# nrclaudio/spVIPES

Measured on AMD Instinct MI355X. Metric: cells/sec/training-step (2-group PoE VAE), higher is better.
Workload: dtype bf16

## Files before the change

include/spvipes_hip.h:

```cpp
#ifndef SPVIPES_HIP_H
#define SPVIPES_HIP_H

#include <stdint.h>

#ifdef __cplusplus
extern "C" {
#endif

#define SPV_OK 0
#define SPV_ERR_ARG (-1)
#define SPV_ERR_LAUNCH (-2)
#define SPV_ERR_UNSUPPORTED (-3)

#define SPV_COUNT_F32 0
#define SPV_COUNT_U16 1

#define SPV_NB_CMAX 64
#define SPV_DEC_KP 16
#define SPV_DEC_KS 32
#define SPV_DEC_KP_WIDE 32
#define SPV_DEC_KS_WIDE 64
#define SPV_DEC_CELLS_PER_WG 128

int spv_version(void);
// ... 263 lines not shown
int spv_bn_bwd(const spv_bn_batch* a, void* stream);

typedef struct spv_sample_prob {
  const float* post; int32_t n;
  const float* eps;
  float* scale; float* logz; float* theta; float* kl;
  const float* g_loc; const float* g_logvar; const float* g_scale; const float* g_logz; const float* g_kl;
  float* d_post;
  int64_t g_ld;
} spv_sample_prob;
typedef struct spv_sample_batch { spv_sample_prob p[SPV_MAXP]; int32_t nprob, B; } spv_sample_batch;
int spv_enc_sample_fwd(const spv_sample_batch* a, void* stream);
int spv_enc_sample_bwd(const spv_sample_batch* a, void* stream);
int spv_enc_heads_fwd(const spv_bn_batch* bn, const spv_sample_batch* sb, void* stream);
int spv_enc_heads_bwd(const spv_bn_batch* bn, const spv_sample_batch* sb, void* stream);

#define SPV_NB_GSPL_MAX 160
#define SPV_POE_LMAX 1024

int spv_poe_partner(const float* labels0, const float* labels1, int32_t B0, int32_t B1, int32_t* order0, int32_t* order1,
                    int32_t* rank0, int32_t* rank1, int32_t* tables, int32_t* partner0, int32_t* mode0,
                    int32_t* partner1, int32_t* mode1, int32_t* err, void* stream);

int spv_poe_rank(const float* labels0, const float* labels1, int32_t B0, int32_t B1, int32_t* order0, int32_t* order1,
                 int32_t* rank0, int32_t* rank1, int32_t* tables, int32_t* err, void* stream);

typedef struct spv_poe_args {
  const float* stats[2]; int64_t ld[2];
  const int32_t* partner[2]; const int32_t* mode[2];
  const float* eps[2];
// ... 121 lines not shown
```

spvipes_amd/_abi.py:

```python
from __future__ import annotations

import ctypes as C
import os
from typing import NamedTuple, Optional

import torch

_HERE = os.path.dirname(os.path.abspath(__file__))
LIB_PATH = os.path.join(_HERE, "_lib", "libspvipes_hip.so")

SPV_COUNT_F32, SPV_COUNT_U16 = 0, 1
NB_CMAX, DEC_KP, DEC_KS, DEC_CELLS_PER_WG = 64, 16, 32, 128
DEC_KPS = DEC_KP + DEC_KS


class DecSlots(NamedTuple):
    kslots: int
    KP: int
    KS: int
    KPS: int


DEC_NARROW = DecSlots(0, DEC_KP, DEC_KS, DEC_KPS)
DEC_WIDE = DecSlots(1, 32, 64, 96)
# ... 58 lines not shown


class SpvBnBatch(C.Structure):
    _fields_ = [("p", SpvBnProb * SPV_MAXP), ("nprob", C.c_int32), ("B", C.c_int32), ("training", C.c_int32), ("relu", C.c_int32),
                ("eps", C.c_float), ("momentum", C.c_float)]


class SpvSampleProb(C.Structure):
    _fields_ = [("post", C.c_void_p), ("n", C.c_int32), ("eps", C.c_void_p), ("scale", C.c_void_p), ("logz", C.c_void_p), ("theta", C.c_void_p),
                ("kl", C.c_void_p), ("g_loc", C.c_void_p), ("g_logvar", C.c_void_p), ("g_scale", C.c_void_p), ("g_logz", C.c_void_p),
                ("g_kl", C.c_void_p), ("d_post", C.c_void_p), ("g_ld", C.c_int64)]


class SpvSampleBatch(C.Structure):
    _fields_ = [("p", SpvSampleProb * SPV_MAXP), ("nprob", C.c_int32), ("B", C.c_int32)]


class SpvPoeArgs(C.Structure):
    _fields_ = [("stats", C.c_void_p * 2), ("ld", C.c_int64 * 2), ("partner", C.c_void_p * 2), ("mode", C.c_void_p * 2), ("eps", C.c_void_p * 2),
                ("loc", C.c_void_p * 2), ("logvar", C.c_void_p * 2), ("scale", C.c_void_p * 2), ("logz", C.c_void_p * 2), ("theta", C.c_void_p * 2),
                ("kl", C.c_void_p * 2), ("g_loc", C.c_void_p * 2), ("g_logvar", C.c_void_p * 2), ("g_scale", C.c_void_p * 2),
                ("g_logz", C.c_void_p * 2), ("g_kl", C.c_void_p * 2), ("d_stats", C.c_void_p * 2), ("B", C.c_int32 * 2), ("n", C.c_int32),
                ("clamp_scale", C.c_int32), ("lone_passthrough", C.c_int32), ("expert", C.c_void_p * 2), ("ld_expert", C.c_int64 * 2),
                ("d_expert", C.c_void_p * 2), ("lab", C.c_void_p * 2), ("order", C.c_void_p * 2), ("rank", C.c_void_p * 2), ("tables", C.c_void_p)]


SPV_POE_MAXG, POE_COMP_SEG, POE_COMP_CMAX = 4, 16, 64


class SpvFc1FwdArgs(C.Structure):
# ... 174 lines not shown
    "spv_dec_tables_grouped": (C.c_int, [C.POINTER(SpvDecGroup), C.c_int32, C.c_void_p]),
    "spv_dec_logits_grouped": (C.c_int, [C.POINTER(SpvDecGroup), C.c_int32, C.c_void_p]),
    "spv_dec_lse_grouped": (C.c_int, [C.POINTER(SpvDecGroup), C.c_int32, C.c_void_p]),
    "spv_dec_nb_fwd_grouped": (C.c_int, [C.POINTER(SpvDecGroup), C.c_int32, C.c_int32, C.c_void_p]),
    "spv_dec_heads_bwd_grouped": (C.c_int, [C.POINTER(SpvDecGroup), C.c_int32, C.c_void_p]),
    "spv_gemm_bf16_grouped": (C.c_int, [C.POINTER(SpvGemmArgs), C.c_int32, C.c_void_p]),
    "spv_linear_fwd": (C.c_int, [C.POINTER(SpvLinearBatch), C.c_void_p]),
    "spv_linear_dgrad": (C.c_int, [C.POINTER(SpvLinearBatch), C.c_void_p]),
    "spv_linear_wgrad": (C.c_int, [C.POINTER(SpvLinearBatch), C.c_void_p, C.c_int64, C.c_void_p]),
    "spv_bn_fwd": (C.c_int, [C.POINTER(SpvBnBatch), C.c_void_p]),
    "spv_bn_bwd": (C.c_int, [C.POINTER(SpvBnBatch), C.c_void_p]),
    "spv_enc_sample_fwd": (C.c_int, [C.POINTER(SpvSampleBatch), C.c_void_p]),
    "spv_enc_sample_bwd": (C.c_int, [C.POINTER(SpvSampleBatch), C.c_void_p]),
    "spv_enc_heads_fwd": (C.c_int, [C.POINTER(SpvBnBatch), C.POINTER(SpvSampleBatch), C.c_void_p]),
    "spv_enc_heads_bwd": (C.c_int, [C.POINTER(SpvBnBatch), C.POINTER(SpvSampleBatch), C.c_void_p]),
    "spv_poe_partner": (C.c_int, [C.c_void_p, C.c_void_p, C.c_int32, C.c_int32, C.c_void_p, C.c_void_p, C.c_void_p, C.c_void_p, C.c_void_p,
                                  C.c_void_p, C.c_void_p, C.c_void_p, C.c_void_p, C.c_void_p, C.c_void_p]),
    "spv_poe_rank": (C.c_int, [C.c_void_p, C.c_void_p, C.c_int32, C.c_int32, C.c_void_p, C.c_void_p, C.c_void_p, C.c_void_p, C.c_void_p, C.c_void_p, C.c_void_p]),
    "spv_poe_fuse_fwd": (C.c_int, [C.POINTER(SpvPoeArgs), C.c_void_p]),
    "spv_poe_fuse_bwd": (C.c_int, [C.POINTER(SpvPoeArgs), C.c_void_p]),
    "spv_plan_invmap": (C.c_int, [C.c_void_p, C.c_int32, C.c_void_p, C.c_int32, C.c_void_p, C.c_int32, C.c_void_p, C.c_int32, C.c_void_p]),
    "spv_plan_argmax": (C.c_int, [C.POINTER(SpvPlan), C.c_void_p, C.c_void_p, C.c_void_p, C.c_void_p, C.c_int32, C.c_int32, C.c_void_p,
                                  C.c_void_p, C.c_void_p]),
    "spv_plan_expert_fwd": (C.c_int, [C.POINTER(SpvPlanExpertArgs), C.c_void_p]),
    "spv_plan_expert_bwd": (C.c_int, [C.POINTER(SpvPlanExpertArgs), C.c_void_p]),
    "spv_poe_comp_fwd": (C.c_int, [C.POINTER(SpvPoeCompArgs), C.c_void_p]),
    "spv_poe_comp_bwd": (C.c_int, [C.POINTER(SpvPoeCompArgs), C.c_void_p]),
    "spv_zsplit_fwd": (C.c_int, [C.POINTER(SpvZsplitArgs), C.c_void_p]),
    "spv_zsplit_bwd": (C.c_int, [C.POINTER(SpvZsplitArgs), C.c_void_p]),
    "spv_bn_fold_fwd": (C.c_int, [C.POINTER(SpvFoldBatch), C.c_void_p]),
# ... 96 lines not shown
```

spvipes_amd/build.py:

```python
from __future__ import annotations

import os
import shutil
import subprocess
import sys

HERE = os.path.dirname(os.path.abspath(__file__))
CSRC = os.path.join(HERE, "csrc")
LIBDIR = os.path.join(HERE, "_lib")
LIB = os.path.join(LIBDIR, "libspvipes_hip.so")
SOURCES = ["spv_abi.hip"]
HEADERS = ["spv_common.h", "spv_gemm.h", "spv_fc1.h", "spv_dec_gemm.h", "spv_decoder.h", "spv_dec_expected.h", "spv_de.h", "spv_de_median.h", "spv_small.h", "spv_poe_n.h", os.path.join("..", "..", "include", "spvipes_hip.h")]


FLAGS = [
    "--offload-arch=gfx950", "-O3", "-std=c++17", "-fPIC", "-shared", "-Wno-unused-value",
    "-fno-slp-vectorize",
]


def build_id() -> str:
    import hashlib

    h = hashlib.sha256()
    h.update(" ".join(FLAGS).encode())
    for name in sorted(SOURCES + HEADERS):
        with open(os.path.join(CSRC, name), "rb") as f:
# ... 44 lines not shown
```

spvipes_amd/csrc/spv_abi.hip:

```cpp
#include "../../include/spvipes_hip.h"
#include "spv_common.h"
#include "spv_gemm.h"
#include "spv_fc1.h"
#include "spv_dec_gemm.h"
#include "spv_decoder.h"
#include "spv_dec_expected.h"
#include "spv_de.h"
#include "spv_de_median.h"
#include "spv_small.h"
#include "spv_poe_n.h"

#include <cstdio>
#include <cstdlib>
#include <cstring>

using namespace spv;

static thread_local char g_err[512] = "";
static int fail(int code, const char* fmt, const char* what = "") {
  snprintf(g_err, sizeof(g_err), fmt, what);
  return code;
}
static int launch_status(const char* what) {
  hipError_t e = hipGetLastError();
// ... 1215 lines not shown
    if (q0.Y != sb->p[e].post || q1.Y != sb->p[e].post + n || q0.ldy != 2 * n || q1.ldy != 2 * n)
      return fail(SPV_ERR_ARG, "%s: the BatchNorm outputs must be the two halves of the sampling problem's post [B][2n]", who);
  }
  return SPV_OK;
}
extern "C" int spv_enc_heads_fwd(const spv_bn_batch* bn, const spv_sample_batch* sb, void* stream) {
  int rc = check_heads(bn, sb, "spv_enc_heads_fwd");
  if (rc) return rc;
  for (int i = 0; i < sb->nprob; ++i) if (!sb->p[i].logz || !sb->p[i].theta || !sb->p[i].kl) return fail(SPV_ERR_ARG, "spv_enc_heads_fwd: null output%s");
  hipStream_t s = (hipStream_t)stream;
  const unsigned nb = (bn->B + BN_ROWS - 1) / BN_ROWS;
  if (bn->training) hipLaunchKernelGGL(bn_stats_kernel, dim3(nb, bn->nprob), dim3(256), 0, s, *bn);
  hipLaunchKernelGGL(enc_heads_bn_sample_fwd_kernel, dim3(nb, sb->nprob), dim3(256), 0, s, *bn, *sb);
  return launch_status("spv_enc_heads_fwd");
}
extern "C" int spv_enc_heads_bwd(const spv_bn_batch* bn, const spv_sample_batch* sb, void* stream) {
  int rc = check_heads(bn, sb, "spv_enc_heads_bwd");
  if (rc) return rc;
  for (int i = 0; i < sb->nprob; ++i) if (!sb->p[i].d_post) return fail(SPV_ERR_ARG, "spv_enc_heads_bwd: null output%s");
  for (int i = 0; i < bn->nprob; ++i) {
    const spv_bn_prob& q = bn->p[i];
    if (!q.dX || !q.dgamma || !q.dbeta) return fail(SPV_ERR_ARG, "spv_enc_heads_bwd: null pointer%s");
    const int e = i / 2, n = sb->p[e].n;
    if (q.dY != sb->p[e].d_post + (i & 1) * n || q.lddy != 2 * n) return fail(SPV_ERR_ARG, "spv_enc_heads_bwd: dY must be the halves of d_post [B][2n]%s");
  }
  if (!bn->training) return fail(SPV_ERR_UNSUPPORTED, "spv_enc_heads_bwd: training-mode BatchNorm only (use spv_enc_sample_bwd + spv_bn_bwd)%s");
  hipStream_t s = (hipStream_t)stream;
  const unsigned nb = (bn->B + BN_ROWS - 1) / BN_ROWS;
  hipLaunchKernelGGL(enc_heads_bwd_reduce_kernel, dim3(nb, sb->nprob), dim3(256), 0, s, *bn, *sb);
  hipLaunchKernelGGL(bn_bwd_apply_fin_kernel, dim3(nb, bn->nprob), dim3(256), 0, s, *bn);
// ... 805 lines not shown
```

spvipes_amd/nn_ops.py:

```python
from __future__ import annotations

import ctypes as C
from typing import List, Optional, Sequence

import torch

from . import _abi
from ._abi import SpvBnBatch, SpvLinearBatch, SpvSampleBatch, ptr, stream_ptr


def _lin_batch(B: int, relu: bool = False, drop_p: float = 0.0, seed=0, accumulate: bool = False) -> SpvLinearBatch:
    b = SpvLinearBatch()
    b.nprob, b.B, b.relu, b.drop_p, b.accumulate = 0, B, int(relu), float(drop_p), int(accumulate)
    if isinstance(seed, torch.Tensor):
        b.seed, b.seed_ptr = 0, seed.data_ptr()
    else:
        b.seed, b.seed_ptr = int(seed), None
    return b


def _add_lin(b: SpvLinearBatch, *, N: int, K: int, W=None, X=None, ldx=0, bias=None, Y=None, ldy=0, dY=None, lddy=0, dX=None, lddx=0,
             dW=None, db=None, keep=None, W2=None, n_w2=0) -> None:
    q = b.p[b.nprob]
    q.X, q.ldx, q.W, q.bias, q.Y, q.ldy, q.keep, q.W2, q.n_w2 = X, ldx, W, bias, Y, ldy, keep, W2, n_w2
# ... 25 lines not shown


class EncoderSpec:

    def __init__(self, enc, h1_group: int, h1_col: int):
        self.enc, self.h1_group, self.h1_col = enc, h1_group, h1_col
        self.n = enc.n_topics

    def params(self) -> List[torch.Tensor]:
        e = self.enc
        return [e.fc2.weight, e.fc2.bias, e.mu_encoder[0].weight, e.mu_encoder[0].bias, e.lvar_encoder[0].weight, e.lvar_encoder[0].bias,
                e.mu_encoder[1].weight, e.mu_encoder[1].bias, e.lvar_encoder[1].weight, e.lvar_encoder[1].bias]


N_ENC_PARAMS = 10


class EncoderTails(torch.autograd.Function):

    @staticmethod
    def forward(ctx, specs: Sequence[EncoderSpec], eps: Sequence[torch.Tensor], training: bool, drop_p: float, seed: int, ws, masks, *tensors):
        ctx.set_materialize_grads(False)
        n_groups = max(s.h1_group for s in specs) + 1
        h1 = tensors[:n_groups]
        par = [tensors[n_groups + i * N_ENC_PARAMS: n_groups + (i + 1) * N_ENC_PARAMS] for i in range(len(specs))]
        B, H = h1[0].shape[0], specs[0].enc.fc2.weight.shape[0]
        dev = h1[0].device
        for t in h1:
            if t.dtype != torch.float32 or not t.is_contiguous():
                raise _abi.SpvError("EncoderTails expects contiguous fp32 h1")
        new = lambda *s: torch.empty(*s, dtype=torch.float32, device=dev)
        h2 = [new(B, H) for _ in specs]
        pre = [new(B, 2 * s.n) for s in specs]
        post = [new(B, 2 * s.n) for s in specs]
        stats = [new(2, s.n, 2) for s in specs]
        nblk = -(-B // _abi.BN_ROWS)
        dp = float(drop_p) if training else 0.0
        b = _lin_batch(B, relu=True, drop_p=dp, seed=seed)
        keep_masks = []
        for i, (s, p, y) in enumerate(zip(specs, par, h2)):
            mk = None
            if masks is not None and masks[i] is not None and dp > 0:
                mk = masks[i].to(dev, torch.float32).contiguous()
                if mk.shape != (B, H):
                    raise _abi.SpvError("dropout mask must be [B, n_hidden]")
                keep_masks.append(mk)
            _add_lin(b, N=H, K=H, W=ptr(p[0]), bias=ptr(p[1]), X=_fptr(h1[s.h1_group], s.h1_col), ldx=h1[s.h1_group].shape[1], Y=ptr(y), ldy=H, keep=ptr(mk))
        _abi.call("spv_linear_fwd", C.byref(b), stream_ptr())
        b = _lin_batch(B)
        for s, p, x, y in zip(specs, par, h2, pre):
            _add_lin(b, N=s.n, K=H, W=ptr(p[2]), bias=ptr(p[3]), X=ptr(x), ldx=H, Y=_fptr(y, 0), ldy=2 * s.n)
            _add_lin(b, N=s.n, K=H, W=ptr(p[4]), bias=ptr(p[5]), X=ptr(x), ldx=H, Y=_fptr(y, s.n), ldy=2 * s.n)
        _abi.call("spv_linear_fwd", C.byref(b), stream_ptr())
        bn = SpvBnBatch()
        bn.nprob, bn.B, bn.training, bn.relu, bn.eps, bn.momentum = 0, B, int(training), 0, 1e-5, 0.1
        parts = []
        for s, p, x, y, st in zip(specs, par, pre, post, stats):
            for half, (g, be, mod) in enumerate(((p[6], p[7], s.enc.mu_encoder[1]), (p[8], p[9], s.enc.lvar_encoder[1]))):
                part = ws.get(f"tail_bn_part_{len(parts)}", (nblk, s.n, 2), torch.float32)
                parts.append(part)
                q = bn.p[bn.nprob]
                q.X, q.ldx, q.Y, q.ldy = _fptr(x, half * s.n), 2 * s.n, _fptr(y, half * s.n), 2 * s.n
                q.gamma, q.beta, q.running_mean, q.running_var = ptr(g), ptr(be), ptr(mod.running_mean), ptr(mod.running_var)
                q.stats, q.part, q.N = ptr(st[half]), ptr(part), s.n
                bn.nprob += 1
        scale = [new(B, s.n) for s in specs]
        logz = [new(B, s.n) for s in specs]
        theta = [new(B, s.n) for s in specs]
        kl = [new(B) for _ in specs]
        sb = SpvSampleBatch()
        sb.nprob, sb.B = len(specs), B
        for i, s in enumerate(specs):
            q = sb.p[i]
            q.post, q.n, q.eps, q.scale, q.logz, q.theta, q.kl = ptr(post[i]), s.n, ptr(eps[i].contiguous()), ptr(scale[i]), ptr(logz[i]), ptr(theta[i]), ptr(kl[i])
        _abi.call("spv_enc_heads_fwd", C.byref(bn), C.byref(sb), stream_ptr())
        ctx.specs, ctx.training, ctx.dp, ctx.seed, ctx.ws, ctx.n_groups, ctx.B, ctx.H = specs, training, dp, seed, ws, n_groups, B, H
        ctx.eps = [e.contiguous() for e in eps]
        ctx.save_for_backward(*tensors, *h2, *pre, *post, *stats, *scale)
        outs = []
        for i, s in enumerate(specs):
            outs += [post[i][:, :s.n], post[i][:, s.n:], scale[i], logz[i], theta[i], kl[i]]
            ctx.mark_non_differentiable(theta[i])
        return tuple(outs)

    @staticmethod
    def backward(ctx, *g):
        specs, B, H, ws, n_groups = ctx.specs, ctx.B, ctx.H, ctx.ws, ctx.n_groups
        E = len(specs)
        saved = ctx.saved_tensors
        n_in = n_groups + E * N_ENC_PARAMS
# ... 33 lines not shown
        k = 0
        for i, (s, p) in enumerate(zip(specs, par)):
            for half, (gam, be, mod) in enumerate(((p[6], p[7], s.enc.mu_encoder[1]), (p[8], p[9], s.enc.lvar_encoder[1]))):
                q = bn.p[bn.nprob]
                q.X, q.ldx, q.Y, q.ldy = _fptr(pre[i], half * s.n), 2 * s.n, _fptr(post[i], half * s.n), 2 * s.n
                q.gamma, q.beta, q.running_mean, q.running_var = ptr(gam), ptr(be), ptr(mod.running_mean), ptr(mod.running_var)
                q.stats, q.part, q.N = ptr(stats[i][half]), ptr(ws.get(f"tail_bn_part_{k}", (nblk, s.n, 2), torch.float32)), s.n
                q.dY, q.lddy, q.dX, q.lddx = _fptr(d_post[i], half * s.n), 2 * s.n, _fptr(d_pre[i], half * s.n), 2 * s.n
                q.dgamma, q.dbeta = ptr(d_gb[i][2 * half]), ptr(d_gb[i][2 * half + 1])
                bn.nprob += 1
                k += 1
        if fused:
            _abi.call("spv_enc_heads_bwd", C.byref(bn), C.byref(sb), stream_ptr())
        else:
            _abi.call("spv_bn_bwd", C.byref(bn), stream_ptr())
        dWmu, dbmu, dWlv, dblv = ([pg[i][2][0] for i in range(E)], [pg[i][3][0] for i in range(E)], [pg[i][4][0] for i in range(E)], [pg[i][5][0] for i in range(E)])
        b = _lin_batch(B)
        for i, s in enumerate(specs):
            _add_lin(b, N=s.n, K=H, W=ptr(par[i][2]), X=ptr(h2[i]), ldx=H, dY=_fptr(d_pre[i], 0), lddy=2 * s.n, dW=ptr(dWmu[i]), db=ptr(dbmu[i]))
            _add_lin(b, N=s.n, K=H, W=ptr(par[i][4]), X=ptr(h2[i]), ldx=H, dY=_fptr(d_pre[i], s.n), lddy=2 * s.n, dW=ptr(dWlv[i]), db=ptr(dblv[i]))
        from . import ops as _ops
        wsw = ws if not isinstance(ws, (list, tuple)) else ws[0]
        _wgrad(b, wsw)
        dh2 = [new(B, H) for _ in specs]
        b = _lin_batch(B)
        for i, s in enumerate(specs):
            _add_lin(b, N=2 * s.n, K=H, W=ptr(par[i][2]), W2=ptr(par[i][4]), n_w2=s.n, dY=ptr(d_pre[i]), lddy=2 * s.n, dX=ptr(dh2[i]), lddx=H)
        _abi.call("spv_linear_dgrad", C.byref(b), stream_ptr())
        dW2, db2 = [pg[i][0][0] for i in range(E)], [pg[i][1][0] for i in range(E)]
        covered = [sorted((s.h1_col, s.h1_col + H) for s in specs if s.h1_group == k) for k in range(n_groups)]
        full = [bool(c) and c[0][0] == 0 and c[-1][1] == h1[k].shape[1] and all(c[i][1] == c[i + 1][0] for i in range(len(c) - 1))
                for k, c in enumerate(covered)]
        dh1 = [torch.empty_like(t) if full[k] else torch.zeros_like(t) for k, t in enumerate(h1)]
        bw = _lin_batch(B, relu=True, drop_p=ctx.dp)
        bd = _lin_batch(B, relu=True, drop_p=ctx.dp)
        for i, s in enumerate(specs):
            x, ldx = _fptr(h1[s.h1_group], s.h1_col), h1[s.h1_group].shape[1]
            _add_lin(bw, N=H, K=H, W=ptr(par[i][0]), X=x, ldx=ldx, Y=ptr(h2[i]), ldy=H, dY=ptr(dh2[i]), lddy=H, dW=ptr(dW2[i]), db=ptr(db2[i]))
            _add_lin(bd, N=H, K=H, W=ptr(par[i][0]), Y=ptr(h2[i]), ldy=H, dY=ptr(dh2[i]), lddy=H, dX=_fptr(dh1[s.h1_group], s.h1_col), lddx=ldx)
        _wgrad(bw, wsw)
        _abi.call("spv_linear_dgrad", C.byref(bd), stream_ptr())
        grads: List[Optional[torch.Tensor]] = list(dh1)
        for i in range(E):
            grads += [pg[i][j][1] for j in range(N_ENC_PARAMS)]
        return (None, None, None, None, None, None, None, *grads)


def _loc_logvar_block(loc: torch.Tensor, logvar: torch.Tensor):
    n = loc.shape[1]
    if (loc.dtype == torch.float32 and loc.stride(1) == 1 and logvar.stride(1) == 1 and loc.stride(0) == logvar.stride(0)
            and logvar.data_ptr() == loc.data_ptr() + 4 * n and loc.stride(0) >= 2 * n):
        return loc, loc.data_ptr(), loc.stride(0)
    blk = torch.cat([loc, logvar], dim=1).contiguous()
    return blk, blk.data_ptr(), 2 * n


# ... 295 lines not shown
```

spvipes_amd/ops.py:

```python
from __future__ import annotations

import ctypes as C
import os
from dataclasses import dataclass
from typing import Dict, Optional, Tuple

import torch

from . import _abi
from ._abi import DEC_CELLS_PER_WG, NB_CMAX, SpvCounts, SpvDecParams, check, ptr, round_up, stream_ptr

N_HIDDEN_MIX = 256


@dataclass
class GroupCounts:

    X: torch.Tensor
    G: int
    col_off: int = 0
    resident: bool = False

    def __post_init__(self):
        self._xb = None
# ... 253 lines not shown
DEC_PAIR_SPLITS = os.environ.get("SPV_DEC_PAIR_SPLITS", "1") != "0"
HEADS_DMA = os.environ.get("SPV_HEADS_DMA", "1") != "0"
FUSED_HEADS = os.environ.get("SPV_FUSED_HEADS", "1") != "0"
GSPLIT_WANT = int(os.environ.get("SPV_GSPLIT_WANT", "512"))
FUSED_HEADS_F32 = os.environ.get("SPV_FUSED_HEADS_F32", "1") != "0"
FUSED_DZ = os.environ.get("SPV_FUSED_DZ", "1") != "0"
FUSED_DZ_F32 = os.environ.get("SPV_FUSED_DZ_F32", "1") != "0"
DA_FIXUP = os.environ.get("SPV_DA_FIXUP", "0")
TRUNK_FOLD = os.environ.get("SPV_TRUNK_FOLD", "1") != "0"
FUSED_PACK = os.environ.get("SPV_FUSED_PACK", "1") != "0"
DEFER_WM = os.environ.get("SPV_DEFER_WM", "1") != "0"
DEFER_BC = os.environ.get("SPV_DEFER_BC", "1") != "0"
DZ_ONLY = os.environ.get("SPV_DZ_ONLY", "0") != "0"
FWD_GROUP_STREAMS = os.environ.get("SPV_FWD_GROUP_STREAMS", "1") != "0"
BWD_GROUP_STREAMS = os.environ.get("SPV_BWD_GROUP_STREAMS", "1") != "0"
_PENDING: list = []
_PENDING_KEEP: list = []


def defer(stream, keep=()) -> None:
    if stream not in _PENDING:
        _PENDING.append(stream)
    _PENDING_KEEP.extend(keep)


def join_all_side_streams(device) -> None:
    dev = torch.device(device)
    cur = torch.cuda.current_stream(dev)
    capturing = torch.cuda.is_current_stream_capturing()
    for (idx, _i), st in _SIDE_STREAMS.items():
# ... 277 lines not shown
```

Before: 6.221 million.

## Fuse encoder tail fc2 and mu/logvar heads into one kernel with BN partials

Adds a fused encoder-tail forward kernel that computes the hidden linear (ReLU and dropout), both mean and log-variance heads, and per-block batch-norm partial statistics in one launch, keeping h2 in shared memory. A matching backward kernel chains the head dgrad and the hidden-layer dgrad through LDS. The goal is to cut launches and global round-trips of intermediates in the small-H encoder tail. It is limited to H in 64/128/256 and head width up to 32, falling back to the old path otherwise, and it uses FP32 MFMA.

```diff
diff --git a/include/spvipes_hip.h b/include/spvipes_hip.h
--- a/include/spvipes_hip.h
+++ b/include/spvipes_hip.h
@@ -301,6 +301,29 @@
 int spv_enc_sample_bwd(const spv_sample_batch* a, void* stream);
 int spv_enc_heads_fwd(const spv_bn_batch* bn, const spv_sample_batch* sb, void* stream);
 int spv_enc_heads_bwd(const spv_bn_batch* bn, const spv_sample_batch* sb, void* stream);
+int spv_enc_heads_fwd_from_partials(const spv_bn_batch* bn, const spv_sample_batch* sb, void* stream);
+
+#define SPV_TAIL_MAXE 4
+typedef struct spv_enc_tail_prob {
+  const float* h1; int64_t ldh1;
+  const float* W2; const float* b2;
+  const float* Wmu; const float* bmu; const float* Wlv; const float* blv;
+  float* h2;
+  float* pre;
+  float* part_mu; float* part_lv;
+  const float* d_pre;
+  float* dh2;
+  float* dh1; int64_t lddh1;
+  int32_t n;
+} spv_enc_tail_prob;
+typedef struct spv_enc_tail_batch {
+  spv_enc_tail_prob p[SPV_TAIL_MAXE];
+  int32_t nprob, B, H;
+  float drop_p;
+  uint64_t seed; const uint64_t* seed_ptr;
+} spv_enc_tail_batch;
+int spv_enc_tail_fwd(const spv_enc_tail_batch* a, void* stream);
+int spv_enc_tail_bwd(const spv_enc_tail_batch* a, void* stream);
 
 #define SPV_NB_GSPL_MAX 160
 #define SPV_POE_LMAX 1024
diff --git a/spvipes_amd/_abi.py b/spvipes_amd/_abi.py
--- a/spvipes_amd/_abi.py
+++ b/spvipes_amd/_abi.py
@@ -96,6 +96,20 @@
 
 class SpvSampleBatch(C.Structure):
     _fields_ = [("p", SpvSampleProb * SPV_MAXP), ("nprob", C.c_int32), ("B", C.c_int32)]
+
+
+SPV_TAIL_MAXE = 4
+
+
+class SpvEncTailProb(C.Structure):
+    _fields_ = [("h1", C.c_void_p), ("ldh1", C.c_int64), ("W2", C.c_void_p), ("b2", C.c_void_p), ("Wmu", C.c_void_p), ("bmu", C.c_void_p),
+                ("Wlv", C.c_void_p), ("blv", C.c_void_p), ("h2", C.c_void_p), ("pre", C.c_void_p), ("part_mu", C.c_void_p), ("part_lv", C.c_void_p),
+                ("d_pre", C.c_void_p), ("dh2", C.c_void_p), ("dh1", C.c_void_p), ("lddh1", C.c_int64), ("n", C.c_int32)]
+
+
+class SpvEncTailBatch(C.Structure):
+    _fields_ = [("p", SpvEncTailProb * SPV_TAIL_MAXE), ("nprob", C.c_int32), ("B", C.c_int32), ("H", C.c_int32), ("drop_p", C.c_float),
+                ("seed", C.c_uint64), ("seed_ptr", C.c_void_p)]
 
 
 class SpvPoeArgs(C.Structure):
@@ -300,6 +314,9 @@
     "spv_enc_sample_bwd": (C.c_int, [C.POINTER(SpvSampleBatch), C.c_void_p]),
     "spv_enc_heads_fwd": (C.c_int, [C.POINTER(SpvBnBatch), C.POINTER(SpvSampleBatch), C.c_void_p]),
     "spv_enc_heads_bwd": (C.c_int, [C.POINTER(SpvBnBatch), C.POINTER(SpvSampleBatch), C.c_void_p]),
+    "spv_enc_heads_fwd_from_partials": (C.c_int, [C.POINTER(SpvBnBatch), C.POINTER(SpvSampleBatch), C.c_void_p]),
+    "spv_enc_tail_fwd": (C.c_int, [C.POINTER(SpvEncTailBatch), C.c_void_p]),
+    "spv_enc_tail_bwd": (C.c_int, [C.POINTER(SpvEncTailBatch), C.c_void_p]),
     "spv_poe_partner": (C.c_int, [C.c_void_p, C.c_void_p, C.c_int32, C.c_int32, C.c_void_p, C.c_void_p, C.c_void_p, C.c_void_p, C.c_void_p,
                                   C.c_void_p, C.c_void_p, C.c_void_p, C.c_void_p, C.c_void_p, C.c_void_p]),
     "spv_poe_rank": (C.c_int, [C.c_void_p, C.c_void_p, C.c_int32, C.c_int32, C.c_void_p, C.c_void_p, C.c_void_p, C.c_void_p, C.c_void_p, C.c_void_p, C.c_void_p]),
diff --git a/spvipes_amd/build.py b/spvipes_amd/build.py
--- a/spvipes_amd/build.py
+++ b/spvipes_amd/build.py
@@ -10,7 +10,7 @@
 LIBDIR = os.path.join(HERE, "_lib")
 LIB = os.path.join(LIBDIR, "libspvipes_hip.so")
 SOURCES = ["spv_abi.hip"]
-HEADERS = ["spv_common.h", "spv_gemm.h", "spv_fc1.h", "spv_dec_gemm.h", "spv_decoder.h", "spv_dec_expected.h", "spv_de.h", "spv_de_median.h", "spv_small.h", "spv_poe_n.h", os.path.join("..", "..", "include", "spvipes_hip.h")]
+HEADERS = ["spv_common.h", "spv_gemm.h", "spv_fc1.h", "spv_dec_gemm.h", "spv_decoder.h", "spv_dec_expected.h", "spv_de.h", "spv_de_median.h", "spv_small.h", "spv_enc_tail.h", "spv_poe_n.h", os.path.join("..", "..", "include", "spvipes_hip.h")]
 
 
 FLAGS = [
diff --git a/spvipes_amd/csrc/spv_abi.hip b/spvipes_amd/csrc/spv_abi.hip
--- a/spvipes_amd/csrc/spv_abi.hip
+++ b/spvipes_amd/csrc/spv_abi.hip
@@ -8,6 +8,7 @@
 #include "spv_de.h"
 #include "spv_de_median.h"
 #include "spv_small.h"
+#include "spv_enc_tail.h"
 #include "spv_poe_n.h"
 
 #include <cstdio>
@@ -1253,6 +1254,53 @@
   hipLaunchKernelGGL(enc_heads_bn_sample_fwd_kernel, dim3(nb, sb->nprob), dim3(256), 0, s, *bn, *sb);
   return launch_status("spv_enc_heads_fwd");
 }
+extern "C" int spv_enc_heads_fwd_from_partials(const spv_bn_batch* bn, const spv_sample_batch* sb, void* stream) {
+  int rc = check_heads(bn, sb, "spv_enc_heads_fwd_from_partials");
+  if (rc) return rc;
+  for (int i = 0; i < sb->nprob; ++i) if (!sb->p[i].logz || !sb->p[i].theta || !sb->p[i].kl) return fail(SPV_ERR_ARG, "spv_enc_heads_fwd_from_partials: null output%s");
+  if (!bn->training) return fail(SPV_ERR_ARG, "spv_enc_heads_fwd_from_partials: training-mode statistics only%s");
+  const unsigned nb = (bn->B + BN_ROWS - 1) / BN_ROWS;
+  hipLaunchKernelGGL(enc_heads_bn_sample_fwd_kernel, dim3(nb, sb->nprob), dim3(256), 0, (hipStream_t)stream, *bn, *sb);
+  return launch_status("spv_enc_heads_fwd_from_partials");
+}
+
+static int check_tail(const spv_enc_tail_batch* a, const char* who, bool bwd) {
+  if (!a || a->nprob <= 0 || a->nprob > SPV_TAIL_MAXE || a->B <= 0) return fail(SPV_ERR_ARG, "%s: bad batch", who);
+  if (a->drop_p < 0.f || a->drop_p >= 1.f) return fail(SPV_ERR_ARG, "%s: dropout probability outside [0,1)", who);
+  if (a->H != 64 && a->H != 128 && a->H != 256) return fail(SPV_ERR_UNSUPPORTED, "%s: H must be 64, 128 or 256", who);
+  for (int i = 0; i < a->nprob; ++i) {
+    const spv_enc_tail_prob& q = a->p[i];
+    if (q.n <= 0 || q.n > 32) return fail(SPV_ERR_UNSUPPORTED, "%s: head width outside 1..32", who);
+    if (!q.W2 || !q.Wmu || !q.Wlv || !q.h2) return fail(SPV_ERR_ARG, "%s: null pointer", who);
+    if (bwd ? (!q.d_pre || !q.dh2 || !q.dh1 || q.lddh1 < a->H)
+            : (!q.h1 || !q.b2 || !q.bmu || !q.blv || !q.pre || q.ldh1 < a->H || (q.part_mu == nullptr) != (q.part_lv == nullptr)))
+      return fail(SPV_ERR_ARG, "%s: bad problem", who);
+    const uintptr_t al = (uintptr_t)q.W2 | (uintptr_t)q.Wmu | (uintptr_t)q.Wlv | (bwd ? 0 : ((uintptr_t)q.h1 | (uintptr_t)(q.ldh1 * 4)));
+    if (al & 15) return fail(SPV_ERR_UNSUPPORTED, "%s: operands must be 16-byte aligned", who);
+  }
+  return SPV_OK;
+}
+extern "C" int spv_enc_tail_fwd(const spv_enc_tail_batch* a, void* stream) {
+  int rc = check_tail(a, "spv_enc_tail_fwd", false);
+  if (rc) return rc;
+  hipStream_t s = (hipStream_t)stream;
+  const unsigned E = a->nprob;
+  if (a->H == 64) hipLaunchKernelGGL(enc_tail_fwd_kernel<64>, dim3((a->B + ENC_TAIL_ROWS<64> - 1) / ENC_TAIL_ROWS<64>, E), dim3(256), 0, s, *a);
+  else if (a->H == 128) hipLaunchKernelGGL(enc_tail_fwd_kernel<128>, dim3((a->B + ENC_TAIL_ROWS<128> - 1) / ENC_TAIL_ROWS<128>, E), dim3(256), 0, s, *a);
+  else hipLaunchKernelGGL(enc_tail_fwd_kernel<256>, dim3((a->B + ENC_TAIL_ROWS<256> - 1) / ENC_TAIL_ROWS<256>, E), dim3(256), 0, s, *a);
+  return launch_status("spv_enc_tail_fwd");
+}
+extern "C" int spv_enc_tail_bwd(const spv_enc_tail_batch* a, void* stream) {
+  int rc = check_tail(a, "spv_enc_tail_bwd", true);
+  if (rc) return rc;
+  hipStream_t s = (hipStream_t)stream;
+  const unsigned E = a->nprob;
+  if (a->H == 64) hipLaunchKernelGGL(enc_tail_bwd_kernel<64>, dim3((a->B + ENC_TAIL_ROWS<64> - 1) / ENC_TAIL_ROWS<64>, E), dim3(256), 0, s, *a);
+  else if (a->H == 128) hipLaunchKernelGGL(enc_tail_bwd_kernel<128>, dim3((a->B + ENC_TAIL_ROWS<128> - 1) / ENC_TAIL_ROWS<128>, E), dim3(256), 0, s, *a);
+  else hipLaunchKernelGGL(enc_tail_bwd_kernel<256>, dim3((a->B + ENC_TAIL_ROWS<256> - 1) / ENC_TAIL_ROWS<256>, E), dim3(256), 0, s, *a);
+  return launch_status("spv_enc_tail_bwd");
+}
+
 extern "C" int spv_enc_heads_bwd(const spv_bn_batch* bn, const spv_sample_batch* sb, void* stream) {
   int rc = check_heads(bn, sb, "spv_enc_heads_bwd");
   if (rc) return rc;
diff --git a/spvipes_amd/csrc/spv_enc_tail.h b/spvipes_amd/csrc/spv_enc_tail.h
--- /dev/null
+++ b/spvipes_amd/csrc/spv_enc_tail.h
@@ -0,0 +1,237 @@
+#pragma once
+#include "spv_small.h"
+
+namespace spv {
+
+typedef spv_enc_tail_prob EncTailProb;
+typedef spv_enc_tail_batch EncTailBatch;
+
+template <int H> constexpr int ENC_TAIL_ROWS = (H <= 64) ? 64 : 32;
+
+__device__ __forceinline__ void issue_fence() { __builtin_amdgcn_sched_barrier(0); }
+
+__device__ const uint64_t g_spv_zero64 = 0;
+
+__device__ __forceinline__ void ld8v(const float* p, float (&v)[8]) {
+  const f4v a = *reinterpret_cast<const f4v*>(p), b = *reinterpret_cast<const f4v*>(p + 4);
+#pragma unroll
+  for (int j = 0; j < 4; ++j) { v[j] = a[j]; v[4 + j] = b[j]; }
+}
+
+template <int H>
+__global__ __launch_bounds__(256) void enc_tail_fwd_kernel(EncTailBatch a) {
+  constexpr int TR = ENC_TAIL_ROWS<H>, RH = TR / 32, CW = 4 / RH, NT = (H / 32) / CW, KS = H / 16, LDH = H + 4, LDP = 65, NCMB = 2 * RH;
+  static_assert(BN_ROWS == 32 && (H / 32) % CW == 0, "tile shape");
+  __shared__ __attribute__((aligned(16))) float s_h2[TR * LDH];
+  __shared__ float s_pre[TR * LDP], s_acc[NCMB][256], s_mean[NCMB][32];
+  const EncTailProb& q = a.p[blockIdx.y];
+  const int lane = threadIdx.x & 63, wave = threadIdx.x >> 6, h = lane >> 5, r = lane & 31;
+  const int rh = wave / CW, cw = wave % CW;
+  const int t0 = blockIdx.x * TR;
+  const int n = q.n;
+  const float* xr = q.h1 + (long)min(t0 + 32 * rh + r, a.B - 1) * q.ldh1 + 8 * h;
+  float xa[KS][8];
+#pragma unroll
+  for (int s = 0; s < KS; ++s) ld8v(xr + 16 * s, xa[s]);
+  issue_fence();
+  const int hr = wave >> 1, half = wave & 1;
+  const float* whr = (half ? q.Wlv : q.Wmu) + (long)min(r, n - 1) * H + 8 * h;
+  const float hbias = (half ? q.blv : q.bmu)[min(r, n - 1)];
+  float wh[KS][8];
+  const uint64_t seed_add = *(a.seed_ptr ? a.seed_ptr : &g_spv_zero64);
+#pragma unroll
+  for (int t = 0; t < NT; ++t) {
+    const int col = 32 * (cw + CW * t) + r;
+    const float* wr = q.W2 + (long)col * H + 8 * h;
+    float wb[KS][8];
+#pragma unroll
+    for (int s = 0; s < KS; ++s) ld8v(wr + 16 * s, wb[s]);
+    const float bias = q.b2[col];
+    if (t == NT - 1 && hr < RH) {
+#pragma unroll
+      for (int s = 0; s < KS; ++s) ld8v(whr + 16 * s, wh[s]);
+    }
+    issue_fence();
+    f16v acc;
+#pragma unroll
+    for (int i = 0; i < 16; ++i) acc[i] = 0.f;
+#pragma unroll
+    for (int s = 0; s < KS; ++s) {
+#pragma unroll
+      for (int j = 0; j < 8; ++j) acc = mfma_f32(xa[s][j], wb[s][j], acc);
+    }
+#pragma unroll
+    for (int i = 0; i < 16; ++i) {
+      const int rl = 32 * rh + crow(i, h), b = t0 + rl;
+      float v = acc[i] + bias;
+      v = fmaxf(v, 0.f);
+      if (a.drop_p > 0.f) {
+        const bool keep = dropout_keep(a.seed + seed_add, blockIdx.y, (long)b * H + col, a.drop_p);
+        v = keep ? v * (1.0f / (1.0f - a.drop_p)) : 0.f;
+      }
+      s_h2[rl * LDH + col] = v;
+      if (b < a.B) q.h2[(long)b * H + col] = v;
+    }
+  }
+  lds_barrier();
+  if (hr < RH) {
+    const float* xs = s_h2 + (32 * hr + r) * LDH + 8 * h;
+    f16v acc;
+#pragma unroll
+    for (int i = 0; i < 16; ++i) acc[i] = 0.f;
+#pragma unroll
+    for (int s = 0; s < KS; ++s) {
+      float x[8];
+      ld8v(xs + 16 * s, x);
+#pragma unroll
+      for (int j = 0; j < 8; ++j) acc = mfma_f32(x[j], wh[s][j], acc);
+    }
+    if (r < n) {
+#pragma unroll
+      for (int i = 0; i < 16; ++i) {
+        const int rl = 32 * hr + crow(i, h), b = t0 + rl;
+        const float v = acc[i] + hbias;
+        s_pre[rl * LDP + 32 * half + r] = v;
+        if (b < a.B) q.pre[(long)b * (2 * n) + half * n + r] = v;
+      }
+    }
+  }
+  if (q.part_mu == nullptr) return;
+  lds_barrier();
+  const int NC = pow2_at_least(n), RS = 256 / NC;
+  const int c = threadIdx.x % NC, slot = threadIdx.x / NC;
+#pragma unroll
+  for (int m = 0; m < NCMB; ++m) {
+    const int bb0 = t0 + 32 * (m >> 1), bb1 = min(bb0 + 32, a.B);
+    float s = 0.f;
+    if (c < n) {
+#pragma unroll 4
+      for (int b = bb0 + slot; b < bb1; b += RS) s += s_pre[(b - t0) * LDP + 32 * (m & 1) + c];
+    }
+    s_acc[m][threadIdx.x] = s;
+  }
+  __syncthreads();
+  if (threadIdx.x < n) {
+#pragma unroll
+    for (int m = 0; m < NCMB; ++m) {
+      const int bb0 = t0 + 32 * (m >> 1), bb1 = min(bb0 + 32, a.B);
+      float t = 0.f;
+      for (int k = 0; k < RS; ++k) t += s_acc[m][k * NC + threadIdx.x];
+      s_mean[m][threadIdx.x] = (bb0 < a.B) ? t / (float)(bb1 - bb0) : 0.f;
+    }
+  }
+  __syncthreads();
+#pragma unroll
+  for (int m = 0; m < NCMB; ++m) {
+    const int bb0 = t0 + 32 * (m >> 1), bb1 = min(bb0 + 32, a.B);
+    float m2 = 0.f;
+    if (c < n) {
+      const float mean = s_mean[m][c];
+#pragma unroll 4
+      for (int b = bb0 + slot; b < bb1; b += RS) { const float d = s_pre[(b - t0) * LDP + 32 * (m & 1) + c] - mean; m2 += d * d; }
+    }
+    s_acc[m][threadIdx.x] = m2;
+  }
+  __syncthreads();
+  if (threadIdx.x < n) {
+#pragma unroll
+    for (int m = 0; m < NCMB; ++m) {
+      const int bb0 = t0 + 32 * (m >> 1);
+      if (bb0 >= a.B) continue;
+      float t = 0.f;
+      for (int k = 0; k < RS; ++k) t += s_acc[m][k * NC + threadIdx.x];
+      float* part = (m & 1) ? q.part_lv : q.part_mu;
+      const long blk = (long)blockIdx.x * RH + (m >> 1);
+      part[(blk * n + threadIdx.x) * 2] = s_mean[m][threadIdx.x];
+      part[(blk * n + threadIdx.x) * 2 + 1] = t;
+    }
+  }
+}
+
+template <int H>
+__global__ __launch_bounds__(256) void enc_tail_bwd_kernel(EncTailBatch a) {
+  constexpr int TR = ENC_TAIL_ROWS<H>, RH = TR / 32, CW = 4 / RH, NT = (H / 32) / CW, KS = H / 16, LDH = H + 4, NS = 4;
+  __shared__ __attribute__((aligned(16))) float s_g[TR * LDH];
+  const EncTailProb& q = a.p[blockIdx.y];
+  const int lane = threadIdx.x & 63, wave = threadIdx.x >> 6, h = lane >> 5, r = lane & 31;
+  const int rh = wave / CW, cw = wave % CW;
+  const int t0 = blockIdx.x * TR;
+  const int n = q.n, N = 2 * n;
+  const float sc = (a.drop_p > 0.f) ? 1.0f / (1.0f - a.drop_p) : 1.0f;
+  const float* gr = q.d_pre + (long)min(t0 + 32 * rh + r, a.B - 1) * N;
+  float ga[NS][8];
+#pragma unroll
+  for (int s = 0; s < NS; ++s) {
+#pragma unroll
+    for (int j = 0; j < 8; ++j) { const int i = 16 * s + 8 * h + j; const bool ok = i < N; const float t = gr[ok ? i : 0]; ga[s][j] = ok ? t : 0.f; }
+  }
+  constexpr bool EARLY_W2 = H <= 128;
+  float w2[KS][8];
+  auto fetch_w2 = [&](int t) {
+    const float* wc = q.W2 + 32 * (cw + CW * t) + r;
+#pragma unroll
+    for (int s = 0; s < KS; ++s) {
+#pragma unroll
+      for (int j = 0; j < 8; ++j) w2[s][j] = wc[(long)(16 * s + 8 * h + j) * H];
+    }
+  };
+  if constexpr (EARLY_W2) fetch_w2(0);
+#pragma unroll
+  for (int t = 0; t < NT; ++t) {
+    const int col = 32 * (cw + CW * t) + r;
+    float wb[NS][8];
+#pragma unroll
+    for (int s = 0; s < NS; ++s) {
+#pragma unroll
+      for (int j = 0; j < 8; ++j) {
+        const int i = 16 * s + 8 * h + j;
+        const bool ok = i < N;
+        const float v = *((i < n) ? q.Wmu + (long)(ok ? i : 0) * H + col : q.Wlv + (long)(ok ? i - n : 0) * H + col);
+        wb[s][j] = ok ? v : 0.f;
+      }
+    }
+    float y[16];
+#pragma unroll
+    for (int i = 0; i < 16; ++i) y[i] = q.h2[(long)min(t0 + 32 * rh + crow(i, h), a.B - 1) * H + col];
+    f16v acc;
+#pragma unroll
+    for (int i = 0; i < 16; ++i) acc[i] = 0.f;
+#pragma unroll
+    for (int s = 0; s < NS; ++s) {
+      if (16 * s < N) {
+#pragma unroll
+        for (int j = 0; j < 8; ++j) acc = mfma_f32(ga[s][j], wb[s][j], acc);
+      }
+    }
+#pragma unroll
+    for (int i = 0; i < 16; ++i) {
+      const int rl = 32 * rh + crow(i, h), b = t0 + rl;
+      s_g[rl * LDH + col] = (y[i] > 0.f) ? acc[i] * sc : 0.f;
+      if (b < a.B) q.dh2[(long)b * H + col] = acc[i];
+    }
+  }
+  lds_barrier();
+  const float* gs = s_g + (32 * rh + r) * LDH + 8 * h;
+#pragma unroll
+  for (int t = 0; t < NT; ++t) {
+    if (t > 0 || !EARLY_W2) fetch_w2(t);
+    const int col = 32 * (cw + CW * t) + r;
+    f16v acc;
+#pragma unroll
+    for (int i = 0; i < 16; ++i) acc[i] = 0.f;
+#pragma unroll
+    for (int s = 0; s < KS; ++s) {
+      float g[8];
+      ld8v(gs + 16 * s, g);
+#pragma unroll
+      for (int j = 0; j < 8; ++j) acc = mfma_f32(g[j], w2[s][j], acc);
+    }
+#pragma unroll
+    for (int i = 0; i < 16; ++i) {
+      const int b = t0 + 32 * rh + crow(i, h);
+      if (b < a.B) q.dh1[(long)b * q.lddh1 + col] = acc[i];
+    }
+  }
+}
+
+}
diff --git a/spvipes_amd/nn_ops.py b/spvipes_amd/nn_ops.py
--- a/spvipes_amd/nn_ops.py
+++ b/spvipes_amd/nn_ops.py
@@ -1,12 +1,13 @@
 from __future__ import annotations
 
 import ctypes as C
+import logging
 from typing import List, Optional, Sequence
 
 import torch
 
 from . import _abi
-from ._abi import SpvBnBatch, SpvLinearBatch, SpvSampleBatch, ptr, stream_ptr
+from ._abi import SpvBnBatch, SpvEncTailBatch, SpvLinearBatch, SpvSampleBatch, ptr, stream_ptr
 
 
 def _lin_batch(B: int, relu: bool = False, drop_p: float = 0.0, seed=0, accumulate: bool = False) -> SpvLinearBatch:
@@ -63,6 +64,48 @@
 
 
 N_ENC_PARAMS = 10
+
+
+TAIL_PATHS: dict = {}
+_log = logging.getLogger(__name__)
+
+
+def _tail_path(reason: str) -> bool:
+    if reason not in TAIL_PATHS and reason not in ("fused", "switched off"):
+        _log.debug("EncoderTails keeps the per-layer launches: %s", reason)
+    TAIL_PATHS[reason] = TAIL_PATHS.get(reason, 0) + 1
+    return reason == "fused"
+
+
+def _tail_fused(specs, par, h1, H: int) -> bool:
+    from . import ops as _ops
+    if not _ops.ENC_TAIL_FUSED:
+        return _tail_path("switched off")
+    if H not in (64, 128, 256) or len(specs) > _abi.SPV_TAIL_MAXE or any(not (0 < s.n <= 32) for s in specs):
+        return _tail_path("shape (H, head width or encoder count)")
+    if any(t.shape[1] % 4 or t.data_ptr() % 16 for t in h1) or any(s.h1_col % 4 or s.h1_col + H > h1[s.h1_group].shape[1] for s in specs):
+        return _tail_path("h1 alignment")
+    for p in par:
+        if any(t.dtype != torch.float32 or not t.is_contiguous() for t in p[:6]) or any(p[j].data_ptr() % 16 for j in (0, 2, 4)):
+            return _tail_path("parameter dtype / layout / alignment")
+        if p[0].shape != (H, H):
+            return _tail_path("shape (H, head width or encoder count)")
+    return True
+
+
+def _tail_batch(specs, par, h1, h2, B: int, H: int, drop_p: float, seed) -> SpvEncTailBatch:
+    b = SpvEncTailBatch()
+    b.nprob, b.B, b.H, b.drop_p = len(specs), B, H, float(drop_p)
+    if isinstance(seed, torch.Tensor):
+        b.seed, b.seed_ptr = 0, seed.data_ptr()
+    else:
+        b.seed, b.seed_ptr = int(seed), None
+    for i, (s, p) in enumerate(zip(specs, par)):
+        q = b.p[i]
+        q.h1, q.ldh1 = _fptr(h1[s.h1_group], s.h1_col), h1[s.h1_group].shape[1]
+        q.W2, q.b2, q.Wmu, q.bmu, q.Wlv, q.blv = (ptr(p[j]) for j in range(6))
+        q.h2, q.n = ptr(h2[i]), s.n
+    return b
 
 
 class EncoderTails(torch.autograd.Function):
@@ -85,22 +128,35 @@
         stats = [new(2, s.n, 2) for s in specs]
         nblk = -(-B // _abi.BN_ROWS)
         dp = float(drop_p) if training else 0.0
-        b = _lin_batch(B, relu=True, drop_p=dp, seed=seed)
-        keep_masks = []
-        for i, (s, p, y) in enumerate(zip(specs, par, h2)):
-            mk = None
-            if masks is not None and masks[i] is not None and dp > 0:
-                mk = masks[i].to(dev, torch.float32).contiguous()
-                if mk.shape != (B, H):
-                    raise _abi.SpvError("dropout mask must be [B, n_hidden]")
-                keep_masks.append(mk)
-            _add_lin(b, N=H, K=H, W=ptr(p[0]), bias=ptr(p[1]), X=_fptr(h1[s.h1_group], s.h1_col), ldx=h1[s.h1_group].shape[1], Y=ptr(y), ldy=H, keep=ptr(mk))
-        _abi.call("spv_linear_fwd", C.byref(b), stream_ptr())
-        b = _lin_batch(B)
-        for s, p, x, y in zip(specs, par, h2, pre):
-            _add_lin(b, N=s.n, K=H, W=ptr(p[2]), bias=ptr(p[3]), X=ptr(x), ldx=H, Y=_fptr(y, 0), ldy=2 * s.n)
-            _add_lin(b, N=s.n, K=H, W=ptr(p[4]), bias=ptr(p[5]), X=ptr(x), ldx=H, Y=_fptr(y, s.n), ldy=2 * s.n)
-        _abi.call("spv_linear_fwd", C.byref(b), stream_ptr())
+        mks = [None] * len(specs)
+        if masks is not None and dp > 0:
+            for i, m in enumerate(masks):
+                if m is not None:
+                    mks[i] = m.to(dev, torch.float32).contiguous()
+                    if mks[i].shape != (B, H):
+                        raise _abi.SpvError("dropout mask must be [B, n_hidden]")
+        fused = _tail_path("injected dropout masks") if any(m is not None for m in mks) else (_tail_fused(specs, par, h1, H) and _tail_path("fused"))
+        tb = None
+        if fused:
+            tb = _tail_batch(specs, par, h1, h2, B, H, dp, seed)
+            for i, (s, x) in enumerate(zip(specs, pre)):
+                q = tb.p[i]
+                q.pre = ptr(x)
+                if training:
+                    q.part_mu = ptr(ws.get(f"tail_bn_part_{2 * i}", (nblk, s.n, 2), torch.float32))
+                    q.part_lv = ptr(ws.get(f"tail_bn_part_{2 * i + 1}", (nblk, s.n, 2), torch.float32))
+            _abi.call("spv_enc_tail_fwd", C.byref(tb), stream_ptr())
+        else:
+            b = _lin_batch(B, relu=True, drop_p=dp, seed=seed)
+            for i, (s, p, y) in enumerate(zip(specs, par, h2)):
+                mk = mks[i]
+                _add_lin(b, N=H, K=H, W=ptr(p[0]), bias=ptr(p[1]), X=_fptr(h1[s.h1_group], s.h1_col), ldx=h1[s.h1_group].shape[1], Y=ptr(y), ldy=H, keep=ptr(mk))
+            _abi.call("spv_linear_fwd", C.byref(b), stream_ptr())
+            b = _lin_batch(B)
+            for s, p, x, y in zip(specs, par, h2, pre):
+                _add_lin(b, N=s.n, K=H, W=ptr(p[2]), bias=ptr(p[3]), X=ptr(x), ldx=H, Y=_fptr(y, 0), ldy=2 * s.n)
+                _add_lin(b, N=s.n, K=H, W=ptr(p[4]), bias=ptr(p[5]), X=ptr(x), ldx=H, Y=_fptr(y, s.n), ldy=2 * s.n)
+            _abi.call("spv_linear_fwd", C.byref(b), stream_ptr())
         bn = SpvBnBatch()
         bn.nprob, bn.B, bn.training, bn.relu, bn.eps, bn.momentum = 0, B, int(training), 0, 1e-5, 0.1
         parts = []
@@ -122,7 +178,8 @@
         for i, s in enumerate(specs):
             q = sb.p[i]
             q.post, q.n, q.eps, q.scale, q.logz, q.theta, q.kl = ptr(post[i]), s.n, ptr(eps[i].contiguous()), ptr(scale[i]), ptr(logz[i]), ptr(theta[i]), ptr(kl[i])
-        _abi.call("spv_enc_heads_fwd", C.byref(bn), C.byref(sb), stream_ptr())
+        _abi.call("spv_enc_heads_fwd_from_partials" if (fused and training) else "spv_enc_heads_fwd", C.byref(bn), C.byref(sb), stream_ptr())
+        ctx.tail_fused = fused
         ctx.specs, ctx.training, ctx.dp, ctx.seed, ctx.ws, ctx.n_groups, ctx.B, ctx.H = specs, training, dp, seed, ws, n_groups, B, H
         ctx.eps = [e.contiguous() for e in eps]
         ctx.save_for_backward(*tensors, *h2, *pre, *post, *stats, *scale)
@@ -186,32 +243,41 @@
             _abi.call("spv_enc_heads_bwd", C.byref(bn), C.byref(sb), stream_ptr())
         else:
             _abi.call("spv_bn_bwd", C.byref(bn), stream_ptr())
-        dWmu, dbmu, dWlv, dblv = ([pg[i][2][0] for i in range(E)], [pg[i][3][0] for i in range(E)], [pg[i][4][0] for i in range(E)], [pg[i][5][0] for i in range(E)])
-        b = _lin_batch(B)
-        for i, s in enumerate(specs):
-            _add_lin(b, N=s.n, K=H, W=ptr(par[i][2]), X=ptr(h2[i]), ldx=H, dY=_fptr(d_pre[i], 0), lddy=2 * s.n, dW=ptr(dWmu[i]), db=ptr(dbmu[i]))
-            _add_lin(b, N=s.n, K=H, W=ptr(par[i][4]), X=ptr(h2[i]), ldx=H, dY=_fptr(d_pre[i], s.n), lddy=2 * s.n, dW=ptr(dWlv[i]), db=ptr(dblv[i]))
         from . import ops as _ops
         wsw = ws if not isinstance(ws, (list, tuple)) else ws[0]
-        _wgrad(b, wsw)
+        dWmu, dbmu, dWlv, dblv = ([pg[i][2][0] for i in range(E)], [pg[i][3][0] for i in range(E)], [pg[i][4][0] for i in range(E)], [pg[i][5][0] for i in range(E)])
+        dW2, db2 = [pg[i][0][0] for i in range(E)], [pg[i][1][0] for i in range(E)]
         dh2 = [new(B, H) for _ in specs]
-        b = _lin_batch(B)
-        for i, s in enumerate(specs):
-            _add_lin(b, N=2 * s.n, K=H, W=ptr(par[i][2]), W2=ptr(par[i][4]), n_w2=s.n, dY=ptr(d_pre[i]), lddy=2 * s.n, dX=ptr(dh2[i]), lddx=H)
-        _abi.call("spv_linear_dgrad", C.byref(b), stream_ptr())
-        dW2, db2 = [pg[i][0][0] for i in range(E)], [pg[i][1][0] for i in range(E)]
         covered = [sorted((s.h1_col, s.h1_col + H) for s in specs if s.h1_group == k) for k in range(n_groups)]
         full = [bool(c) and c[0][0] == 0 and c[-1][1] == h1[k].shape[1] and all(c[i][1] == c[i + 1][0] for i in range(len(c) - 1))
                 for k, c in enumerate(covered)]
         dh1 = [torch.empty_like(t) if full[k] else torch.zeros_like(t) for k, t in enumerate(h1)]
+        bh = _lin_batch(B)
         bw = _lin_batch(B, relu=True, drop_p=ctx.dp)
-        bd = _lin_batch(B, relu=True, drop_p=ctx.dp)
         for i, s in enumerate(specs):
+            _add_lin(bh, N=s.n, K=H, W=ptr(par[i][2]), X=ptr(h2[i]), ldx=H, dY=_fptr(d_pre[i], 0), lddy=2 * s.n, dW=ptr(dWmu[i]), db=ptr(dbmu[i]))
+            _add_lin(bh, N=s.n, K=H, W=ptr(par[i][4]), X=ptr(h2[i]), ldx=H, dY=_fptr(d_pre[i], s.n), lddy=2 * s.n, dW=ptr(dWlv[i]), db=ptr(dblv[i]))
             x, ldx = _fptr(h1[s.h1_group], s.h1_col), h1[s.h1_group].shape[1]
             _add_lin(bw, N=H, K=H, W=ptr(par[i][0]), X=x, ldx=ldx, Y=ptr(h2[i]), ldy=H, dY=ptr(dh2[i]), lddy=H, dW=ptr(dW2[i]), db=ptr(db2[i]))
-            _add_lin(bd, N=H, K=H, W=ptr(par[i][0]), Y=ptr(h2[i]), ldy=H, dY=ptr(dh2[i]), lddy=H, dX=_fptr(dh1[s.h1_group], s.h1_col), lddx=ldx)
-        _wgrad(bw, wsw)
-        _abi.call("spv_linear_dgrad", C.byref(bd), stream_ptr())
+        if ctx.tail_fused:
+            tb = _tail_batch(specs, par, h1, h2, B, H, ctx.dp, 0)
+            for i, s in enumerate(specs):
+                q = tb.p[i]
+                q.d_pre, q.dh2, q.dh1, q.lddh1 = ptr(d_pre[i]), ptr(dh2[i]), _fptr(dh1[s.h1_group], s.h1_col), h1[s.h1_group].shape[1]
+            _abi.call("spv_enc_tail_bwd", C.byref(tb), stream_ptr())
+            _wgrad(bh, wsw)
+            _wgrad(bw, wsw)
+        else:
+            _wgrad(bh, wsw)
+            b = _lin_batch(B)
+            for i, s in enumerate(specs):
+                _add_lin(b, N=2 * s.n, K=H, W=ptr(par[i][2]), W2=ptr(par[i][4]), n_w2=s.n, dY=ptr(d_pre[i]), lddy=2 * s.n, dX=ptr(dh2[i]), lddx=H)
+            _abi.call("spv_linear_dgrad", C.byref(b), stream_ptr())
+            bd = _lin_batch(B, relu=True, drop_p=ctx.dp)
+            for i, s in enumerate(specs):
+                _add_lin(bd, N=H, K=H, W=ptr(par[i][0]), Y=ptr(h2[i]), ldy=H, dY=ptr(dh2[i]), lddy=H, dX=_fptr(dh1[s.h1_group], s.h1_col), lddx=h1[s.h1_group].shape[1])
+            _wgrad(bw, wsw)
+            _abi.call("spv_linear_dgrad", C.byref(bd), stream_ptr())
         grads: List[Optional[torch.Tensor]] = list(dh1)
         for i in range(E):
             grads += [pg[i][j][1] for j in range(N_ENC_PARAMS)]
diff --git a/spvipes_amd/ops.py b/spvipes_amd/ops.py
--- a/spvipes_amd/ops.py
+++ b/spvipes_amd/ops.py
@@ -291,6 +291,7 @@
 DZ_ONLY = os.environ.get("SPV_DZ_ONLY", "0") != "0"
 FWD_GROUP_STREAMS = os.environ.get("SPV_FWD_GROUP_STREAMS", "1") != "0"
 BWD_GROUP_STREAMS = os.environ.get("SPV_BWD_GROUP_STREAMS", "1") != "0"
+ENC_TAIL_FUSED = os.environ.get("SPV_ENC_TAIL_FUSED", "1") != "0"
 _PENDING: list = []
 _PENDING_KEEP: list = []
 
```

Measured after the change: 6.297 million, median of 5. +1.2%, better.
